# ku222/Attention-GAN

Hardware: AMD Instinct MI355X
Metric: train images/sec at 256×256 stage-3, batch 24/GPU, 1/2/4/8 MI355X (higher is better)
Workload: dtype f32; 1 GPU; full 3-stage AttnGAN 64->128->256 train step: G + 3xD updates + word attention + DAMSM words/sentence loss + KL + 4x fused Adam (BASELINE.json configs[2]); workload_key=full3, batch_per_gpu=24, global_batch=24, gf_dim=32, df_dim=64, emb_dim=256, seq_len=10, text_encoder=bypassed (frozen; N(0,1) embeddings), parallelism=dp1, discriminator_streams=3, launch=eager, gradient_exchange=none (one rank), losses_finite=True

## Files before the change

attention-gan_amd/csrc/conv.hip:

```cpp
#include "conv_common.h"

#include <cxxabi.h>
#include <cstdlib>


using namespace agan;

using namespace agan::conv;

namespace {

__global__ __launch_bounds__(256) void ktable_kernel(int2* __restrict__ tab, int n, int K, int RS, int S, int IHW, int IW, int DY) {
    const int k = blockIdx.x * 256 + threadIdx.x;
    if (k >= n) return;
    int2 a, b;
    if (k < K) {
        const int c = k / RS, rs = k - c * RS, r = rs / S, q = rs - r * S;
        const int dy = r * DY, dx = q * DY;
        a.x = c * IHW + dy * IW + dx;
        a.y = (dy & 0xFFFF) | (dx << 16);
        b.x = c * IHW * 4;
        b.y = rs * kTapRowBytes;
    } else {
        a.x = 0;
// ... 693 lines not shown
        const int kt = cdiv(K, 64);
        pack_fwd_tile(j.w, wk, j.cout, K, Nld, local % kt, local / kt, reinterpret_cast<float (*)[65]>(buf));
    } else if (j.mode == AGAN_PACK_DGRAD_S1 && j.kh * j.kw <= 16) {
        const int cg = cdiv(j.cout, kPackCo);
        pack_dgrad_tile<AGAN_PACK_DGRAD_S1>(j.w, wk, j.cout, j.cin, j.kh, j.kw, Nld, local % cg, local / cg, buf, true);
    } else if (j.mode == AGAN_PACK_DGRAD_4x4S2) {
        const int cg = cdiv(j.cout, kPackCo);
        pack_dgrad_tile<AGAN_PACK_DGRAD_4x4S2>(j.w, wk, j.cout, j.cin, j.kh, j.kw, Nld, local % cg, local / cg, buf, true);
    } else {
        const int nb = pack_job_blocks(j.mode, j.cout, j.cin, j.kh, j.kw);
        const size_t total = (size_t)ncls * K * Nld;
        for (size_t e = (size_t)local * 256 + threadIdx.x; e < total; e += (size_t)nb * 256) {
            const int n = (int)(e % Nld);
            const size_t t = e / Nld;
            wk[e] = packed_weight_value(j.w, j.mode, (int)(t / K), (int)(t % K), n, j.cout, j.cin, j.kh, j.kw);
        }
    }
}

__global__ __launch_bounds__(256) void unpack_wgrad_up_kernel(const float* __restrict__ dwk, float* __restrict__ dw, int cout, int cin,
                                                              int accumulate) {
    const int K = cin * 4;
    const size_t total = (size_t)cout * cin * 9;
    for (size_t e = (size_t)blockIdx.x * blockDim.x + threadIdx.x; e < total; e += (size_t)gridDim.x * blockDim.x) {
        const int ab = (int)(e % 9), a = ab / 3, b = ab - a * 3;
        const size_t t = e / 9;
        const int ci = (int)(t % cin), co = (int)(t / cin);
        float v = 0.f;
        for (int py = 0; py < 2; ++py)
            for (int r = 0; r < 2; ++r) {
                int rl, rh;
                up_fwd_taps(py, r, rl, rh);
                if (a < rl || a > rh) continue;
                for (int px = 0; px < 2; ++px)
                    for (int q = 0; q < 2; ++q) {
                        int sl, sh;
                        up_fwd_taps(px, q, sl, sh);
                        if (b < sl || b > sh) continue;
                        v += dwk[((size_t)(py * 2 + px) * cout + co) * K + (ci * 4 + r * 2 + q)];
                    }
            }
        dw[e] = accumulate ? dw[e] + v : v;
    }
}

__global__ __launch_bounds__(256) void bias_grad_kernel(const float* __restrict__ dy, float* __restrict__ db, int B, int C,
                                                        int HW, int accumulate) {
    __shared__ float red[4];
    const int c = blockIdx.x;
    float s = 0.f;
    for (int b = 0; b < B; ++b) {
        const float* p = dy + ((size_t)b * C + c) * HW;
        for (int i = threadIdx.x; i < HW; i += 256) s += p[i];
    }
    s = block_sum<256>(s, red);
    if (threadIdx.x == 0) db[c] = accumulate ? db[c] + s : s;
}

}

static thread_local hipEvent_t g_timer_start = nullptr, g_timer_stop = nullptr;
static thread_local const void* g_timed_kernel = nullptr;
static thread_local int g_timed_split = 0;
namespace agan { namespace conv { thread_local const void* g_noted_kernel = nullptr; } }
static inline void timer_begin(hipStream_t st) {
    if (g_timer_start) (void)hipEventRecord(g_timer_start, st);
}
static inline void timer_end(hipStream_t st, int split) {
    if (g_timer_stop) {
        (void)hipEventRecord(g_timer_stop, st);
        g_timed_kernel = agan::conv::g_noted_kernel;
        g_timed_split = split;
    }
    g_timer_start = g_timer_stop = nullptr;
}
namespace agan { namespace conv {
void timed_begin(hipStream_t st) { timer_begin(st); }
void timed_end(hipStream_t st, int split) { timer_end(st, split); }
} }

static bool dt16(int dt) { return dt == AGAN_DT_BF16 || dt == AGAN_DT_F16; }
static int mode_dtype(int mode) { return mode == AGAN_PREC_BF16 ? AGAN_DT_BF16 : (mode == AGAN_PREC_F16 ? AGAN_DT_F16 : AGAN_DT_F32); }

enum class GatherPath { none, p16, patch, winograd, small_n, direct };
struct GatherRoute {
    int mode = AGAN_PREC_F32;
    GatherPath path = GatherPath::none;
    P16Plan p16{};
    PatchPlan pp{};
    PatchGather patch{};
    WinoPlan wino{};
    GatherPlan direct{};
    size_t ws_bytes = 0;
    int split = 1;
};

static GatherRoute route_gather(const agan_conv_geom* gg, int prec, int in_dtype, int out_dtype, bool epilogue) {
    GatherRoute r;
    auto take = [&r](GatherPath path, size_t ws_bytes, int split) {
        r.path = path;
        r.ws_bytes = ws_bytes;
        r.split = split;
        return r;
    };
    if (check_geom(gg)) return r;
    const Geom g = make_geom(gg);
    if (prec_planes(prec) > 0 && patch_supported(g)) r.mode = prec;
    const bool f32io = in_dtype == AGAN_DT_F32 && out_dtype == AGAN_DT_F32;
    if (const int want = mode_dtype(r.mode)) {
        if ((in_dtype == AGAN_DT_F32 || in_dtype == want) && (out_dtype == AGAN_DT_F32 || out_dtype == want)) {
            r.p16 = plan_p16(g, in_dtype != AGAN_DT_F32);
            if (r.p16.ok) return take(GatherPath::p16, r.p16.ws_bytes, r.p16.ksplit);
        }
    }
    if (r.mode != AGAN_PREC_F32) {
        if (!f32io) return r;
        r.pp = make_patch_plan(g);
        r.patch = plan_patch_gather(g, r.pp);
        return take(GatherPath::patch, r.patch.ws_bytes, r.patch.ksplit);
    }
    if (f32io && !epilogue) {
        r.wino = plan_wino(g);
        if (r.wino.ok) return take(GatherPath::winograd, r.wino.ws_bytes, r.wino.ksplit);
    }
    if (small_n_gather_supported(g)) {
        const bool linear = g.RS == 1 && g.IH == 1 && g.IW == 1;
        if ((in_dtype == AGAN_DT_F32 || (dt16(in_dtype) && !linear)) && out_dtype == AGAN_DT_F32) return take(GatherPath::small_n, 0, 1);
        return r;
    }
    if (in_dtype == AGAN_DT_F32 && (out_dtype == AGAN_DT_F32 || dt16(out_dtype))) {
        r.direct = plan_gather(g, AGAN_PREC_F32);
        return take(GatherPath::direct, r.direct.ws_bytes, r.direct.ksplit);
    }
    return r;
}

enum class WgradPath { none, winograd, rows, patch, small_n, direct };
struct WgradRoute {
    int mode = AGAN_PREC_F32;
    WgradPath path = WgradPath::none;
    WinoWgradPlan wino{};
    RowsPlan rows{};
    PatchPlan pp{};
    PatchWgrad patch{};
    SmallWgradPlan small{};
    WgradPlan direct{};
    size_t ws_bytes = 0;
    int split = 1;
};

static WgradRoute route_wgrad(const agan_conv_geom* gg, int pack_mode, int prec, int x_dtype, int dy_dtype) {
    WgradRoute r;
    auto take = [&r](WgradPath path, size_t ws_bytes, int split) {
        r.path = path;
        r.ws_bytes = ws_bytes;
        r.split = split;
        return r;
    };
    if (check_geom(gg)) return r;
    const Geom g = make_geom(gg);
    const bool up = pack_mode == AGAN_PACK_UP_FWD, x16 = x_dtype != AGAN_DT_F32, y16 = dy_dtype != AGAN_DT_F32;
    if (prec_planes(prec) > 0 && patch_supported(g)) {
        r.mode = prec;
        if (prec == AGAN_PREC_BF16X6) r.mode = AGAN_PREC_F16X3;
        if (up && !plan_rows_wgrad(g, r.mode, false, false, true).ok) r.mode = AGAN_PREC_F32;
    }
    if (x16 || y16) {
        const int want = mode_dtype(r.mode);
        const bool ok = r.mode == AGAN_PREC_F32
                            ? pack_mode == AGAN_PACK_FWD && small_n_wgrad_supported(g) && dt16(x_dtype) && !y16
                            : want != AGAN_DT_F32 && (!x16 || x_dtype == want) && (!y16 || dy_dtype == want);
        if (!ok) return r;
    }
    if (r.mode == AGAN_PREC_F32 && !up && !x16 && !y16) {
        r.wino = plan_wino_wgrad(g);
        if (r.wino.ok) return take(WgradPath::winograd, r.wino.ws_bytes, r.wino.psplit);
    }
    if (!(r.mode == AGAN_PREC_F32 && small_n_wgrad_supported(g))) {
        r.rows = plan_rows_wgrad(g, r.mode, x16, y16, up);
        if (r.rows.ok) return take(WgradPath::rows, r.rows.ws_bytes, r.rows.psplit);
    }
    if (r.mode != AGAN_PREC_F32) {
        r.pp = make_patch_plan(g);
        r.patch = plan_patch_wgrad(g, r.pp, r.mode);
        return take(WgradPath::patch, r.patch.ws_bytes, r.patch.psplit);
    }
    if (!up && small_n_wgrad_supported(g)) {
        r.small = plan_wgrad_small_n(g);
        return take(WgradPath::small_n, r.small.ws_bytes, r.small.nchunk);
    }
    if (!x16 && !y16) {
        r.direct = plan_wgrad(g, up);
        return take(WgradPath::direct, r.direct.ws_bytes, r.direct.psplit);
    }
    return r;
}

static int check_ws(const char* who, size_t need, const void* ws, size_t ws_bytes) {
    if (need > ws_bytes || (need && !ws)) {
        set_error("%s: workspace %zu < %zu", who, ws_bytes, need);
        return AGAN_EWORKSPACE;
    }
    return AGAN_OK;
}

template <class Launch>
static int launch_main(hipStream_t st, int split, const char* what, Launch&& launch) {
    timer_begin(st);
    launch();
    timer_end(st, split);
    return check_launch(what);
}

extern "C" {

int agan_timer_last_kernel(char* name, size_t capacity) {
    AGAN_REQUIRE(name && capacity > 1, "timer_last_kernel: bad argument");
    name[0] = 0;
    if (!g_timed_kernel) return AGAN_OK;
    const char* mangled = hipKernelNameRefByPtr(g_timed_kernel, nullptr);
    if (!mangled) return AGAN_OK;
    int status = 0;
    char* dem = abi::__cxa_demangle(mangled, nullptr, nullptr, &status);
    const char* src = (status == 0 && dem) ? dem : mangled;
    strncpy(name, src, capacity - 1);
    name[capacity - 1] = 0;
    free(dem);
    return AGAN_OK;
}

int agan_timer_last_split(void) { return g_timed_kernel ? g_timed_split : 0; }

int agan_timer_create(void** event) {
    AGAN_REQUIRE(event != nullptr, "timer_create: null pointer");
    hipEvent_t e;
    if (hipEventCreate(&e) != hipSuccess) {
        set_error("timer_create: hipEventCreate failed");
        return AGAN_ELAUNCH;
    }
    *event = e;
    return AGAN_OK;
}
int agan_timer_destroy(void* event) { return (event && hipEventDestroy(static_cast<hipEvent_t>(event)) != hipSuccess) ? AGAN_ELAUNCH : AGAN_OK; }
int agan_timer_arm(void* start, void* stop) {
    g_timer_start = static_cast<hipEvent_t>(start);
    g_timer_stop = static_cast<hipEvent_t>(stop);
    return AGAN_OK;
}
int agan_timer_elapsed_ms(void* start, void* stop, float* ms) {
    AGAN_REQUIRE(start && stop && ms, "timer_elapsed_ms: null pointer");
    if (hipEventElapsedTime(ms, static_cast<hipEvent_t>(start), static_cast<hipEvent_t>(stop)) != hipSuccess) {
        set_error("timer_elapsed_ms: events not complete");
        return AGAN_ELAUNCH;
    }
    return AGAN_OK;
}

size_t agan_packed_weight_bytes(int mode, int cout, int cin, int kh, int kw, int prec) {
    int ncls, K, N;
    if (pack_dims(mode, cout, cin, kh, kw, ncls, K, N)) return 0;
    if (prec == AGAN_PREC_F32) return (size_t)ncls * K * ((N + 31) / 32 * 32) * sizeof(float);
    if (mode == AGAN_PACK_DGRAD_3x3S2) return 0;
    if (prec_planes(prec) > 0) return patch_packed_weight_bytes(mode, cout, cin, kh, kw, prec);
    return 0;
}

int agan_pack_weight(const float* w, void* wkv, int mode, int cout, int cin, int kh, int kw, int prec, void* stream) {
    int ncls, K, N;
    AGAN_REQUIRE(w && wkv, "pack_weight: null pointer");
    AGAN_REQUIRE(prec == AGAN_PREC_F32 || prec_planes(prec) > 0, "pack_weight: unknown precision mode %d", prec);
    if (prec != AGAN_PREC_F32) {
        AGAN_REQUIRE(mode != AGAN_PACK_DGRAD_3x3S2, "pack_weight: AGAN_PACK_DGRAD_3x3S2 has an fp32 layout only");
        AGAN_REQUIRE(pack_dims(mode, cout, cin, kh, kw, ncls, K, N) == 0, "pack_weight: mode %d does not take %dx%d", mode, kh, kw);
        return pack_weight_patch(w, wkv, mode, cout, cin, kh, kw, prec, as_stream(stream));
    }
    float* wk = static_cast<float*>(wkv);
    AGAN_REQUIRE(pack_dims(mode, cout, cin, kh, kw, ncls, K, N) == 0, "pack_weight: mode %d does not take %dx%d", mode, kh, kw);
    const int Nld = ((N + 31) / 32 * 32);
    const size_t total = (size_t)ncls * K * Nld;
    const int blocks = (int)std::min<size_t>(cdivz(total, 256), 8192);
    hipStream_t pst = as_stream(stream);
    if (mode == AGAN_PACK_FWD) {
        AGAN_LAUNCH(pack_fwd_tiled_kernel, dim3(cdiv(K, 64), cdiv(Nld, 64)), dim3(256), 0, pst, w, wk, cout, K, Nld);
        return check_launch("pack_weight/fwd");
    }
    if ((mode == AGAN_PACK_DGRAD_S1 && kh * kw <= 16) || mode == AGAN_PACK_DGRAD_4x4S2) {
        if (Nld != cin) (void)hipMemsetAsync(wk, 0, total * sizeof(float), pst);
        dim3 grid(cdiv(cout, kPackCo), cdiv(cin, 64));
        if (mode == AGAN_PACK_DGRAD_S1) AGAN_LAUNCH((pack_dgrad_tiled_kernel<AGAN_PACK_DGRAD_S1>), grid, dim3(256), 0, pst, w, wk, cout, cin, kh, kw, Nld);
        else AGAN_LAUNCH((pack_dgrad_tiled_kernel<AGAN_PACK_DGRAD_4x4S2>), grid, dim3(256), 0, pst, w, wk, cout, cin, kh, kw, Nld);
        return check_launch("pack_weight/dgrad");
    }
    AGAN_LAUNCH(pack_weight_kernel, dim3(blocks), dim3(256), 0, as_stream(stream), w, wk, mode, cout, cin, kh, kw, K,
                       Nld, ncls);
    return check_launch("pack_weight");
}

int agan_pack_job_blocks(int mode, int cout, int cin, int kh, int kw) { return pack_job_blocks(mode, cout, cin, kh, kw); }
int agan_pack_job_blocks_prec(int mode, int cout, int cin, int kh, int kw, int prec) {
    return prec == AGAN_PREC_F32 ? pack_job_blocks(mode, cout, cin, kh, kw) : (prec_planes(prec) > 0 ? pack_job_blocks_patch(mode, cout, cin, kh, kw) : 0);
}

int agan_pack_weights(const agan_pack_job* jobs, int njobs, int total_blocks, int prec, void* stream) {
    AGAN_REQUIRE(jobs && njobs > 0 && total_blocks > 0, "pack_weights: empty job list");
    AGAN_REQUIRE(prec == AGAN_PREC_F32 || prec_planes(prec) > 0, "pack_weights: unknown precision mode %d", prec);
    if (prec != AGAN_PREC_F32) return pack_weights_patch(jobs, njobs, total_blocks, prec, as_stream(stream));
    AGAN_LAUNCH(pack_jobs_kernel, dim3(total_blocks), dim3(256), 0, as_stream(stream), jobs, njobs);
    return check_launch("pack_weights");
}

int agan_conv_effective_prec(const agan_conv_geom* g, int prec) { return route_gather(g, prec, AGAN_DT_F32, AGAN_DT_F32, false).mode; }

int agan_conv_wgrad_effective_prec(const agan_conv_geom* g, int pack_mode, int prec) {
    return route_wgrad(g, pack_mode, prec, AGAN_DT_F32, AGAN_DT_F32).mode;
}

double agan_conv_executed_fraction(const agan_conv_geom* g, int prec, int wgrad, int plain_epilogue) {
    if (prec != AGAN_PREC_F32) return 1.0;
    if (wgrad)
        return route_wgrad(g, AGAN_PACK_FWD, prec, AGAN_DT_F32, AGAN_DT_F32).path == WgradPath::winograd ? 16.0 / 36.0 : 1.0;
    const GatherRoute r = route_gather(g, prec, AGAN_DT_F32, AGAN_DT_F32, !plain_epilogue);
    if (r.path != GatherPath::winograd) return 1.0;
    switch (r.wino.kind) {
    case WinoKind::conv4x4_s2: return 36.0 / 64.0;
    case WinoKind::dgrad2x2_class: return 9.0 / 16.0;
    case WinoKind::conv3x3:
    case WinoKind::conv3x3_half: break;
    }
    return 16.0 / 36.0;
}

static const int kDtypes[] = {AGAN_DT_F32, AGAN_DT_BF16, AGAN_DT_F16};

size_t agan_conv_gather_ws_bytes(const agan_conv_geom* g, int prec) {
    size_t a = 0;
    for (int in_dtype : kDtypes)
        for (int out_dtype : kDtypes)
            for (int epilogue = 0; epilogue < 2; ++epilogue) a = std::max(a, route_gather(g, prec, in_dtype, out_dtype, epilogue != 0).ws_bytes);
    return a;
}

size_t agan_conv_ktable_elems(const agan_conv_geom* g) {
    if (check_geom(g)) return 0;
    return (size_t)ktable_entries(g->Cin * g->R * g->S) * 4;
}

int agan_conv_ktable(const agan_conv_geom* gg, int32_t* table, void* stream) {
    if (int e = check_geom(gg)) return e;
    AGAN_REQUIRE(table != nullptr, "conv_ktable: null pointer");
    const Geom g = make_geom(gg);
    const int n = ktable_entries(g.K);
    AGAN_LAUNCH(ktable_kernel, dim3(cdiv(n, 256)), dim3(256), 0, as_stream(stream), reinterpret_cast<int2*>(table), n, g.K, g.RS,
                       g.S, g.IH * g.IW, g.IW, g.DY);
    return check_launch("conv_ktable");
}

int agan_conv_gather_dt_supported(const agan_conv_geom* gg, int prec, int in_dtype, int out_dtype) {
    return route_gather(gg, prec, in_dtype, out_dtype, false).path != GatherPath::none ? 1 : 0;
}

int agan_conv_gather_dt(const void* in_v, const void* wkv, const float* bias, void* out_v, const agan_conv_geom* gg, const int32_t* ktable,
                        int prec, int act, const void* lrelu_mask_v, void* ws, size_t ws_bytes, void* stream, const float* in_scale,
                        float* out_amax, int in_dtype, int out_dtype) {
    if (int e = check_geom(gg)) return e;
    AGAN_REQUIRE(in_v && wkv && out_v && ktable, "conv_gather: null pointer");
    AGAN_REQUIRE(act == AGAN_ACT_NONE || (act == AGAN_ACT_LRELU && gg->Cout > 4),
                 "conv_gather: fused activation %d not available for this call (MFMA paths, LeakyReLU only)", act);
    AGAN_REQUIRE(!lrelu_mask_v || (gg->Cout > 4 && act == AGAN_ACT_NONE),
                 "conv_gather: the LeakyReLU-derivative mask needs an MFMA path and no other activation");
    AGAN_REQUIRE(prec == AGAN_PREC_F32 || prec_planes(prec) > 0, "conv_gather: unknown precision mode %d", prec);
    const GatherRoute r = route_gather(gg, prec, in_dtype, out_dtype, bias || act != AGAN_ACT_NONE || lrelu_mask_v);
    AGAN_REQUIRE(r.mode == prec,
                 "conv_gather: precision mode %d does not take this geometry (agan_conv_effective_prec says which one does)", prec);
    AGAN_REQUIRE(r.path != GatherPath::none,
                 "conv_gather: 16-bit activation storage (%d -> %d) is not available for this geometry / precision %d "
                 "(agan_conv_gather_dt_supported)", in_dtype, out_dtype, prec);
    AGAN_REQUIRE(prec != AGAN_PREC_F16X3 || in_scale != nullptr, "conv_gather: AGAN_PREC_F16X3 needs the operand's agan_absmax_scale pair");
    if (int e = check_ws("conv_gather", r.ws_bytes, ws, ws_bytes)) return e;
    const Geom g = make_geom(gg);
    hipStream_t st = as_stream(stream);
    const float* in = static_cast<const float*>(in_v);
    const float* wk = static_cast<const float*>(wkv);
    const float* lrelu_mask = static_cast<const float*>(lrelu_mask_v);
    void* dst = r.split > 1 ? ws : out_v;
    const float* slabs = static_cast<const float*>(ws);
    size_t slab = 0;
    float* sum_amax = nullptr;
    int e = AGAN_OK;
    switch (r.path) {
        case GatherPath::p16:
            slab = r.p16.slab;
            e = launch_main(st, r.split, "conv_gather/p16", [&] {
                launch_p16_gather(in_v, wkv, bias, dst, g, r.p16, prec, act, lrelu_mask_v, st, in_dtype != AGAN_DT_F32, out_dtype != AGAN_DT_F32);
            });
            break;
        case GatherPath::patch:
            slab = r.patch.slab;
            sum_amax = out_amax;
            e = launch_main(st, r.split, "conv_gather/patch", [&] {
                launch_patch_gather(in, wkv, bias, static_cast<float*>(dst), g, r.pp, r.patch, prec, act, lrelu_mask, st, in_scale, out_amax);
            });
            break;
        case GatherPath::winograd:
            slab = r.wino.slab;
            slabs = reinterpret_cast<const float*>(static_cast<const char*>(ws) + r.wino.u_bytes);
            e = launch_main(st, r.split, "conv_gather/winograd", [&] { launch_wino(in, wk, static_cast<float*>(out_v), g, r.wino, ws, st); });
            break;
        case GatherPath::small_n:
            e = launch_main(st, r.split, "conv_gather/small_n", [&] { launch_gather_small_n(in_v, wk, bias, static_cast<float*>(out_v), g, st, in_dtype); });
            break;
        default: {
            const GatherPlan& p = r.direct;
            slab = p.slab;
            const int2* ktab = reinterpret_cast<const int2*>(ktable);
            e = launch_main(st, r.split, "conv_gather", [&] {
                if (p.bn == 128) launch_gather<128, 2, 2>(in, wk, bias, dst, ktab, g, p, act, lrelu_mask_v, st, out_dtype);
                else if (p.bn == 64) launch_gather<64, 2, 2>(in, wk, bias, dst, ktab, g, p, act, lrelu_mask_v, st, out_dtype);
                else launch_gather<32, 4, 1>(in, wk, bias, dst, ktab, g, p, act, lrelu_mask_v, st, out_dtype);
            });
        }
    }
    if (e || r.split == 1) return e;
    launch_sum_slabs(slabs, r.split, (size_t)g.B * g.Cout * g.OH * g.OW, slab, bias, g.Cout, g.OH * g.OW, out_v, 0, act, lrelu_mask_v, sum_amax, st,
                     out_dtype);
    return check_launch("conv_gather/sum_slabs");
}

int agan_conv_gather(const float* in, const void* wkv, const float* bias, float* out, const agan_conv_geom* gg, const int32_t* ktable,
                     int prec, int act, const float* lrelu_mask, void* ws, size_t ws_bytes, void* stream, const float* in_scale,
                     float* out_amax) {
    return agan_conv_gather_dt(in, wkv, bias, out, gg, ktable, prec, act, lrelu_mask, ws, ws_bytes, stream, in_scale, out_amax,
                               AGAN_DT_F32, AGAN_DT_F32);
}

static const int kPrecs[] = {AGAN_PREC_F32, AGAN_PREC_BF16, AGAN_PREC_BF16X3, AGAN_PREC_F16, AGAN_PREC_BF16X6, AGAN_PREC_F16X3};

size_t agan_conv_wgrad_ws_bytes(const agan_conv_geom* g) {
    if (check_geom(g)) return 0;
    const int pack_mode = g->OS == 2 ? AGAN_PACK_UP_FWD : AGAN_PACK_FWD;
    size_t a = 0;
    for (int prec : kPrecs)
        for (int x_dtype : kDtypes)
            for (int dy_dtype : kDtypes) a = std::max(a, route_wgrad(g, pack_mode, prec, x_dtype, dy_dtype).ws_bytes);
    return a;
}

int agan_conv_wgrad_dt_supported(const agan_conv_geom* gg, int pack_mode, int prec, int x_dtype, int dy_dtype) {
    return route_wgrad(gg, pack_mode, prec, x_dtype, dy_dtype).path != WgradPath::none ? 1 : 0;
}

int agan_conv_wgrad(const float* x, const float* dy, float* dw, const agan_conv_geom* gg, const int32_t* ktable, int pack_mode,
                    int kh, int kw, int prec, int accumulate, void* ws, size_t ws_bytes, void* stream, const float* x_scale,
                    const float* dy_scale) {
    return agan_conv_wgrad_dt(x, dy, dw, gg, ktable, pack_mode, kh, kw, prec, accumulate, ws, ws_bytes, stream, x_scale, dy_scale,
                              AGAN_DT_F32, AGAN_DT_F32);
}

int agan_conv_wgrad_dt(const void* x_v, const void* dy_v, float* dw, const agan_conv_geom* gg, const int32_t* ktable, int pack_mode,
                       int kh, int kw, int prec, int accumulate, void* ws, size_t ws_bytes, void* stream, const float* x_scale,
                       const float* dy_scale, int x_dtype, int dy_dtype) {
    const WgradRoute r = route_wgrad(gg, pack_mode, prec, x_dtype, dy_dtype);
    AGAN_REQUIRE(r.path != WgradPath::none,
                 "conv_wgrad: 16-bit activation storage (%d, %d) is not available for this geometry / precision %d", x_dtype, dy_dtype, prec);
    AGAN_REQUIRE(x_v && dy_v && dw && ktable, "conv_wgrad: null pointer");
    AGAN_REQUIRE(prec == AGAN_PREC_F32 || prec_planes(prec) > 0, "conv_wgrad: unknown precision mode %d", prec);
    AGAN_REQUIRE(pack_mode == AGAN_PACK_FWD || pack_mode == AGAN_PACK_UP_FWD, "conv_wgrad: pack mode %d is not a forward mode", pack_mode);
    const Geom g = make_geom(gg);
    const bool up = pack_mode == AGAN_PACK_UP_FWD;
    AGAN_REQUIRE(1LL * g.B * g.Cin * g.IH * g.IW < (1LL << 29) && 1LL * g.B * g.Cout * g.OH * g.OW < (1LL << 29),
                 "conv_wgrad: tensor exceeds 2^29 elements");
    if (!up) AGAN_REQUIRE(g.R == kh && g.S == kw && g.OS == 1, "conv_wgrad: geometry is not a direct %dx%d conv", kh, kw);
    else AGAN_REQUIRE(g.R == 2 && g.S == 2 && g.OS == 2 && kh == 3 && kw == 3, "conv_wgrad: geometry is not the folded upsample conv");
    AGAN_REQUIRE(r.mode != AGAN_PREC_F16X3 || (x_scale && dy_scale),
                 "conv_wgrad: precision mode %d runs this weight gradient as AGAN_PREC_F16X3 (agan_conv_wgrad_effective_prec), which needs the "
                 "amax slots of x and dy (x_amax / dy_amax)", prec);
    if (int e = check_ws("conv_wgrad", r.ws_bytes, ws, ws_bytes)) return e;
    hipStream_t st = as_stream(stream);
    const float* x = static_cast<const float*>(x_v);
    const float* dy = static_cast<const float*>(dy_v);
    float* wsf = static_cast<float*>(ws);
    const bool x16 = x_dtype != AGAN_DT_F32, y16 = dy_dtype != AGAN_DT_F32;
    switch (r.path) {
        case WgradPath::winograd:
            if (int e = launch_main(st, r.split, "conv_wgrad/winograd", [&] { launch_wino_wgrad(x, dy, wsf, g, r.wino, st); })) return e;
            launch_wino_wgrad_sum(wsf, g, r.wino, dw, accumulate ? 1 : 0, st);
            return check_launch("conv_wgrad/winograd/sum");
        case WgradPath::rows:
        case WgradPath::patch: {
            const bool rows = r.path == WgradPath::rows;
            int e;
            if (rows) e = launch_main(st, r.split, "conv_wgrad/rows", [&] {
                launch_rows_wgrad(x_v, dy_v, wsf, g, r.rows, r.mode, st, x_scale, dy_scale, x16, y16);
            });
            else e = launch_main(st, r.split, "conv_wgrad/patch", [&] {
                launch_patch_wgrad(x_v, dy_v, wsf, g, r.pp, r.patch, r.mode, st, x_scale, dy_scale, x16, y16);
            });
            if (e) return e;
            const size_t slab = rows ? r.rows.slab : r.patch.slab;
            const int NPH = rows ? r.rows.NPH : r.pp.NPH, NT = rows ? r.rows.NT : r.pp.NT, Kp = rows ? r.rows.Kp : r.patch.Kp;
            const int ncls = rows ? 1 : r.patch.ncls;
            const bool unfold = up && !rows;
            float* reduced = r.split > 1 ? wsf + slab * r.split : wsf;
            const bool sum_first = unfold ? r.split > 1 : r.split > 4;
            if (sum_first) {
                launch_sum_slabs(wsf, r.split, (size_t)ncls * g.Cout * Kp, slab, nullptr, 1, 1, reduced, 0, AGAN_ACT_NONE, nullptr, nullptr, st);
                if (int e2 = check_launch("conv_wgrad/sum_slabs")) return e2;
            }
            if (unfold) launch_patch_wgrad_unpack(reduced, dw, g.Cout, g.Cin, kh, kw, up, r.pp, r.patch, accumulate, st);
            else launch_wgrad_sum_unpack(sum_first ? reduced : wsf, sum_first ? 1 : r.split, slab, dw, g.Cout, g.Cin, kh, kw, NPH, NT, Kp, accumulate, st);
            return check_launch("conv_wgrad/unpack");
        }
        case WgradPath::small_n: {
            if (int e = launch_main(st, r.split, "conv_wgrad/small_n", [&] { launch_wgrad_small_n(x_v, dy, wsf, g, r.small, st, x_dtype); })) return e;
            launch_sum_slabs(wsf, r.split, (size_t)g.Cout * g.K, r.small.slab, nullptr, 1, 1, dw, accumulate, AGAN_ACT_NONE, nullptr, nullptr, st);
            return check_launch("conv_wgrad/small_n/sum_slabs");
        }
        default: {
            const WgradPlan& p = r.direct;
            const int acc_in_kernel = (accumulate && !up && p.psplit == 1) ? 1 : 0;
            const bool via_sum = p.psplit > 1 || (accumulate && !up && !acc_in_kernel);
            float* reduced = up ? wsf + (p.psplit > 1 ? p.slab * p.psplit : 0) : dw;
            float* part = via_sum ? wsf : reduced;
            const int2* ktab = reinterpret_cast<const int2*>(ktable);
            dim3 grid(p.itiles, p.jtiles, p.ncls * p.psplit);
#define AGAN_WG(BI, BJ) AGAN_LAUNCH((conv_wgrad_f32_kernel<BI, BJ>), grid, dim3(256), 0, st, x, dy, part, ktab, g, p.psplit, p.pchunk, p.slab, acc_in_kernel)
            const int e = launch_main(st, r.split, "conv_wgrad", [&] {
                if (p.bi == 128 && p.bj == 128) AGAN_WG(128, 128);
                else if (p.bi == 128) AGAN_WG(128, 64);
                else if (p.bj == 128) AGAN_WG(64, 128);
                else AGAN_WG(64, 64);
            });
#undef AGAN_WG
            if (e) return e;
            if (via_sum) {
                launch_sum_slabs(part, p.psplit, (size_t)p.ncls * g.Cout * g.K, p.slab, nullptr, 1, 1, reduced, (accumulate && !up) ? 1 : 0,
                                 AGAN_ACT_NONE, nullptr, nullptr, st);
                if (int e2 = check_launch("conv_wgrad/sum_slabs")) return e2;
            }
            if (up) {
                const size_t total = (size_t)g.Cout * g.Cin * 9;
                AGAN_LAUNCH(unpack_wgrad_up_kernel, dim3((unsigned)std::min<size_t>(cdivz(total, 256), 4096)), dim3(256), 0, st,
                            reduced, dw, g.Cout, g.Cin, accumulate);
                return check_launch("conv_wgrad/unpack");
            }
            return AGAN_OK;
        }
    }
}

int agan_bias_grad(const float* dy, float* dbias, int B, int C, int HW, int accumulate, void* stream) {
    AGAN_REQUIRE(dy && dbias && B > 0 && C > 0 && HW > 0, "bias_grad: bad argument");
    AGAN_LAUNCH(bias_grad_kernel, dim3(C), dim3(256), 0, as_stream(stream), dy, dbias, B, C, HW, accumulate);
    return check_launch("bias_grad");
}

static int conv2d_geom(const agan_conv2d_desc* d, int dgrad, Geom& g, int& pack_mode) {
    AGAN_REQUIRE(d != nullptr, "conv2d: null descriptor");
    AGAN_REQUIRE(d->B > 0 && d->Cin > 0 && d->IH > 0 && d->IW > 0 && d->Cout > 0 && d->OH > 0 && d->OW > 0, "conv2d: non-positive dimension");
    AGAN_REQUIRE(d->KH > 0 && d->KW > 0 && d->KH * d->KW <= kMaxTaps2d, "conv2d: %dx%d taps unsupported (at most %d)", d->KH, d->KW, kMaxTaps2d);
    AGAN_REQUIRE((d->SH == 1 || d->SH == 2) && (d->SW == 1 || d->SW == 2), "conv2d: strides %dx%d unsupported (1 or 2 per axis)", d->SH, d->SW);
    AGAN_REQUIRE(d->PH >= 0 && d->PW >= 0 && d->PH < d->KH && d->PW < d->KW, "conv2d: padding %dx%d unsupported for %dx%d taps", d->PH, d->PW,
                 d->KH, d->KW);
    AGAN_REQUIRE(d->OH == (d->IH + 2 * d->PH - d->KH) / d->SH + 1 && d->OW == (d->IW + 2 * d->PW - d->KW) / d->SW + 1 &&
                     d->IH + 2 * d->PH >= d->KH && d->IW + 2 * d->PW >= d->KW,
                 "conv2d: output %dx%d does not match input %dx%d, taps %dx%d, stride %dx%d, padding %dx%d", d->OH, d->OW, d->IH, d->IW, d->KH,
                 d->KW, d->SH, d->SW, d->PH, d->PW);
    AGAN_REQUIRE(d->in_c0 >= 0 && d->in_c0 + d->Cin <= d->in_ctot && d->out_c0 >= 0 && d->out_c0 + d->Cout <= d->out_ctot,
                 "conv2d: channel slice out of range (in %d+%d of %d, out %d+%d of %d)", d->in_c0, d->Cin, d->in_ctot, d->out_c0, d->Cout,
                 d->out_ctot);
    const long long xe = 1LL * d->B * d->in_ctot * d->IH * d->IW, ye = 1LL * d->B * d->out_ctot * d->OH * d->OW;
    AGAN_REQUIRE(xe < (1LL << 30) && ye < (1LL << 30), "conv2d: tensor exceeds 2^30 elements (32-bit buffer offsets)");
    Geom& r = g;
    r = Geom{};
    r.B = d->B;
    r.DY = 1;
    const int xhw = d->IH * d->IW, yhw = d->OH * d->OW;
    if (!dgrad) {
        r.Cin = d->Cin; r.IH = d->IH; r.IW = d->IW; r.Cout = d->Cout; r.OH = d->OH; r.OW = d->OW;
        r.R = d->KH; r.S = d->KW; r.OS = 1; r.SY = d->SH; r.SX = d->SW;
        r.OY0 = r.OY1 = -d->PH; r.OX0 = r.OX1 = -d->PW;
        r.in0 = d->in_c0 * xhw; r.inB = d->in_ctot * xhw; r.out0 = d->out_c0 * yhw; r.outB = d->out_ctot * yhw;
        pack_mode = AGAN_PACK_FWD;
    } else {
        r.Cin = d->Cout; r.IH = d->OH; r.IW = d->OW; r.Cout = d->Cin; r.OH = d->IH; r.OW = d->IW;
        r.in0 = d->out_c0 * yhw; r.inB = d->out_ctot * yhw; r.out0 = d->in_c0 * xhw; r.outB = d->in_ctot * xhw;
        r.SY = r.SX = 1;
        if (d->SH == 1 && d->SW == 1) {
            r.R = d->KH; r.S = d->KW; r.OS = 1;
            r.OY0 = r.OY1 = -(d->KH - 1 - d->PH); r.OX0 = r.OX1 = -(d->KW - 1 - d->PW);
            pack_mode = AGAN_PACK_DGRAD_S1;
        } else {
            AGAN_REQUIRE(d->SH == 2 && d->SW == 2 && d->KH == 3 && d->KW == 3 && d->PH == 0 && d->PW == 0,
                         "conv2d: no data-gradient decomposition for %dx%d taps, stride %dx%d, padding %dx%d (stride 2: 3x3 unpadded only)",
                         d->KH, d->KW, d->SH, d->SW, d->PH, d->PW);
// ... 78 lines not shown
```

attention-gan_amd/csrc/conv_common.h:

```cpp
#pragma once
#include "agan_common.h"

#include <algorithm>
#include <type_traits>

namespace agan {
namespace conv {

typedef float f32x16 __attribute__((ext_vector_type(16)));

extern thread_local const void* g_noted_kernel;
#define AGAN_LAUNCH(kernel, ...)                                                   \
    do {                                                                           \
        ::agan::conv::g_noted_kernel = reinterpret_cast<const void*>(kernel);      \
        hipLaunchKernelGGL(kernel, __VA_ARGS__);                                   \
    } while (0)
void timed_begin(hipStream_t st);
void timed_end(hipStream_t st, int split);


struct FastDiv {
    unsigned mul, shift;
    __device__ __forceinline__ int div(int n) const { return (int)((__umulhi(mul, (unsigned)n) + (unsigned)n) >> shift); }
};
// ... 128 lines not shown
__host__ __device__ inline int pack_dims(int mode, int cout, int cin, int kh, int kw, int& ncls, int& K, int& N) {
    switch (mode) {
        case AGAN_PACK_FWD: ncls = 1; K = cin * kh * kw; N = cout; return 0;
        case AGAN_PACK_DGRAD_S1: ncls = 1; K = cout * kh * kw; N = cin; return 0;
        case AGAN_PACK_DGRAD_4x4S2: if (kh != 4 || kw != 4) return -1; ncls = 4; K = cout * 4; N = cin; return 0;
        case AGAN_PACK_UP_FWD: if (kh != 3 || kw != 3) return -1; ncls = 4; K = cin * 4; N = cout; return 0;
        case AGAN_PACK_UP_DGRAD: if (kh != 3 || kw != 3) return -1; ncls = 1; K = cout * 16; N = cin; return 0;
        case AGAN_PACK_DGRAD_3x3S2: if (kh != 3 || kw != 3) return -1; ncls = 4; K = cout * 4; N = cin; return 0;
    }
    return -1;
}

__device__ __forceinline__ int linear_block_id() { return blockIdx.x + gridDim.x * (blockIdx.y + gridDim.y * blockIdx.z); }
__device__ __forceinline__ int xcd_contiguous(int L, int T) {
    const int xcd = L & 7, idx = L >> 3;
    int start = 0;
    for (int i = 0; i < xcd; ++i) start += (T - i + 7) >> 3;
    return start + idx;
}

struct GatherPlan {
    int bn, mtiles, ntiles, ncls, ksplit, kchunk;
    size_t slab, ws_bytes;
};

inline GatherPlan plan_gather(const Geom& g, int prec) {
    const int bk = prec == AGAN_PREC_F32 ? 16 : 32;
    const int slots = prec == AGAN_PREC_F32 ? 768 : 512;
    GatherPlan p;
    p.bn = g.Cout >= 96 ? 128 : (g.Cout >= 48 ? 64 : 32);
    p.mtiles = cdiv(g.Mtot, 128);
    p.ntiles = cdiv(g.Cout, p.bn);
    p.ncls = g.OS * g.OS;
    const int tiles = p.mtiles * p.ntiles * p.ncls;
    const int ktiles = cdiv(g.K, bk);
    int ks = 1;
    if (tiles < slots) ks = std::max(1, std::min({slots / tiles, std::max(1, ktiles / 16), 32}));
    p.kchunk = cdiv(ktiles, ks) * bk;
    p.ksplit = cdiv(g.K, p.kchunk);
    p.slab = (size_t)g.B * g.Cout * g.OH * g.OW;
    p.slab = (p.slab + 3) / 4 * 4;
    p.ws_bytes = p.ksplit > 1 ? p.slab * p.ksplit * sizeof(float) : 0;
    return p;
}

struct WgradPlan {
    int bi, bj, itiles, jtiles, ncls, psplit, pchunk;
    size_t slab, ws_bytes;
};

inline WgradPlan plan_wgrad(const Geom& g, bool needs_combine) {
    WgradPlan p;
    p.bi = (g.K >= 96 && cdiv(g.K, 128) * 128 <= cdiv(g.K, 64) * 64) ? 128 : 64;
    p.bj = g.Cout >= 96 ? 128 : 64;
    p.itiles = cdiv(g.K, p.bi);
    p.jtiles = cdiv(g.Cout, p.bj);
    p.ncls = g.OS * g.OS;
    const int tiles = p.itiles * p.jtiles * p.ncls;
    const int ptiles = cdiv(g.Mtot, 32);
    int ps = 1;
    if (tiles < 512) {
        const int cap = std::max(1, ptiles / 4);
        const int ps1 = std::max(1, std::min(512 / tiles, cap)), ps2 = std::max(1, std::min(1024 / tiles, cap));
        const double fill1 = (double)tiles * ps1 / 512.0, fill2 = (double)tiles * ps2 / 1024.0;
        ps = std::min(fill2 > fill1 + 1e-9 ? ps2 : ps1, 2048);
    }
    p.pchunk = cdiv(ptiles, ps) * 32;
    p.psplit = cdiv(g.Mtot, p.pchunk);
    p.slab = ((size_t)p.ncls * g.Cout * g.K + 3) / 4 * 4;
    const size_t nslabs = p.psplit + (needs_combine ? 1 : 0);
    p.ws_bytes = p.slab * nslabs * sizeof(float);
    return p;
}

struct SmallWgradPlan {
    int pchunk, nchunk;
    size_t slab, ws_bytes;
};
bool small_n_gather_supported(const Geom& g);
void launch_gather_small_n(const void* in, const float* wk, const float* bias, float* out, const Geom& g, hipStream_t st, int in_dtype = AGAN_DT_F32);
bool small_n_wgrad_supported(const Geom& g);
SmallWgradPlan plan_wgrad_small_n(const Geom& g);
void launch_wgrad_small_n(const void* x, const float* dy, float* part, const Geom& g, const SmallWgradPlan& p, hipStream_t st, int x_dtype = AGAN_DT_F32);

__host__ __device__ inline void pack_taps(int mode, int kh, int kw, int& R, int& S, int& SY) {
    switch (mode) {
        case AGAN_PACK_DGRAD_4x4S2: case AGAN_PACK_UP_FWD: R = S = 2; SY = 1; return;
        case AGAN_PACK_UP_DGRAD: R = S = 4; SY = 2; return;
        default: R = kh; S = kw; SY = (kh == 4) ? 2 : 1; return;
    }
}
struct PatchPlan {
    int twl, thl;
    int tiles_x, tiles_y, tiles_b, mtiles;
    int PW, PH, PHW, PP;
    int NPH, NT, IS;
    int nchunks, nstages, nsteps;
    int tapoff[9];
    int tappos[9];
    int base_y[2][2], base_x[2][2];
    FastDiv dPP, dPHW, dPW;
    FastDiv dNT, dNCLS, dMT, dTX, dTY, dNPH, dNPH2;
    int g_ntiles, g_ncls;
};
struct PatchGather {
    int bn, ntiles, ncls, ksplit, stages_per_split;
    size_t slab, ws_bytes;
};
struct PatchWgrad {
    int bj, jtiles, ncls, psplit, tiles_per_split, Kp;
    size_t slab, ws_bytes;
};
struct P16Plan {
    int ok;
    int gk;
    int twl, thl, TB;
    int tiles_x, tiles_y, tiles_b, mtiles;
    int PH, PW, LW, NXB, PXB, CHS;
    int nitems, NI;
    int nstages, wsteps;
    int bn, ntiles, ncls, ksplit, stages_per_split;
    int buf_bytes, smem_bytes;
    int lds_epi;
    int px2;
    int wc, lp;
    size_t slab, ws_bytes;
    FastDiv dNXB, dPH, dTB, dNT, dNCLS, dMT, dTX, dTY;
};
P16Plan plan_p16(const Geom& g, bool in16);
void launch_p16_gather(const void* in, const void* wk, const float* bias, void* dst, const Geom& g, const P16Plan& p, int prec, int act,
                       const void* lrelu_mask, hipStream_t st, bool in16, bool out16);
struct RowsPlan {
    int ok, gk, ci2, ups;
    int twl, thl, tbl;
    int tiles_x, tiles_y, tiles_b, mtiles;
    int XR, XRT;
    int rowb, cpitch;
    int halo, NBY, drowb, dpitch;
    int plane_bytes, smem_bytes, pc;
    int nxbl, nxitems, nyitems;
    int bj, jtiles, nchunks, ngroups, psplit, tiles_per_split;
    int NPH, NT, Kp;
    size_t slab, ws_bytes;
    FastDiv dXRT, dXR, dNBY;
};
enum class WinoKind : int {
    conv3x3,
    conv3x3_half,
    conv4x4_s2,
    dgrad2x2_class,
};
struct WinoPlan {
    int ok;
    WinoKind kind;
    int txl, tyl;
    int blocks_x, blocks_y, blocks_b, mtiles;
    int nf, ntiles;
    int pcp, raw_items, raw_bytes;
    int mpc, mpr;
    int smem_bytes;
    int ksplit, chunks_per_split;
    size_t u_bytes, slab, ws_bytes;
};
struct WinoWgradPlan {
    int ok, noct, jtiles, itiles, psplit, octs_per_split, smem_bytes;
    size_t slab, ws_bytes;
// ... 34 lines not shown
```

Before: 1001 images/s.

## Add skinny fully-connected forward and weight-gradient kernels for small batch

Adds a dedicated path for 1x1-spatial convolutions (linear layers such as the noise/condition FC and the attention projections) with small batch M. The forward kernel stages the whole input batch in LDS, streams weight columns per lane, and splits K across waves and blocks, with an optional combine kernel. The wgrad kernel holds x in registers and writes dW directly with no split-slab workspace. It is meant to replace the generic small_n and direct tiles, which underuse the GPU on tall-skinny GEMMs. In exchange it adds routing complexity and a distinct epilogue class (bias allowed, activation not).

```diff
diff --git a/attention-gan_amd/csrc/conv.hip b/attention-gan_amd/csrc/conv.hip
--- a/attention-gan_amd/csrc/conv.hip
+++ b/attention-gan_amd/csrc/conv.hip
@@ -799,7 +799,7 @@
 static bool dt16(int dt) { return dt == AGAN_DT_BF16 || dt == AGAN_DT_F16; }
 static int mode_dtype(int mode) { return mode == AGAN_PREC_BF16 ? AGAN_DT_BF16 : (mode == AGAN_PREC_F16 ? AGAN_DT_F16 : AGAN_DT_F32); }
 
-enum class GatherPath { none, p16, patch, winograd, small_n, direct };
+enum class GatherPath { none, p16, patch, winograd, skinny, small_n, direct };
 struct GatherRoute {
     int mode = AGAN_PREC_F32;
     GatherPath path = GatherPath::none;
@@ -807,12 +807,14 @@
     PatchPlan pp{};
     PatchGather patch{};
     WinoPlan wino{};
+    SkinnyGatherPlan skinny{};
     GatherPlan direct{};
     size_t ws_bytes = 0;
     int split = 1;
 };
 
-static GatherRoute route_gather(const agan_conv_geom* gg, int prec, int in_dtype, int out_dtype, bool epilogue) {
+enum { kEpiNone = 0, kEpiBias = 1, kEpiAct = 2 };
+static GatherRoute route_gather(const agan_conv_geom* gg, int prec, int in_dtype, int out_dtype, int epilogue) {
     GatherRoute r;
     auto take = [&r](GatherPath path, size_t ws_bytes, int split) {
         r.path = path;
@@ -836,9 +838,13 @@
         r.patch = plan_patch_gather(g, r.pp);
         return take(GatherPath::patch, r.patch.ws_bytes, r.patch.ksplit);
     }
-    if (f32io && !epilogue) {
+    if (f32io && epilogue == kEpiNone) {
         r.wino = plan_wino(g);
         if (r.wino.ok) return take(GatherPath::winograd, r.wino.ws_bytes, r.wino.ksplit);
+    }
+    if (f32io && epilogue != kEpiAct && skinny_gather_supported(g)) {
+        r.skinny = plan_gather_skinny(g);
+        return take(GatherPath::skinny, r.skinny.ws_bytes, r.skinny.ksplit);
     }
     if (small_n_gather_supported(g)) {
         const bool linear = g.RS == 1 && g.IH == 1 && g.IW == 1;
@@ -852,7 +858,7 @@
     return r;
 }
 
-enum class WgradPath { none, winograd, rows, patch, small_n, direct };
+enum class WgradPath { none, winograd, rows, patch, skinny, small_n, direct };
 struct WgradRoute {
     int mode = AGAN_PREC_F32;
     WgradPath path = WgradPath::none;
@@ -860,6 +866,7 @@
     RowsPlan rows{};
     PatchPlan pp{};
     PatchWgrad patch{};
+    SkinnyWgradPlan skinny{};
     SmallWgradPlan small{};
     WgradPlan direct{};
     size_t ws_bytes = 0;
@@ -902,6 +909,10 @@
         r.patch = plan_patch_wgrad(g, r.pp, r.mode);
         return take(WgradPath::patch, r.patch.ws_bytes, r.patch.psplit);
     }
+    if (!up && !x16 && !y16 && skinny_wgrad_supported(g)) {
+        r.skinny = plan_wgrad_skinny(g);
+        return take(WgradPath::skinny, 0, 1);
+    }
     if (!up && small_n_wgrad_supported(g)) {
         r.small = plan_wgrad_small_n(g);
         return take(WgradPath::small_n, r.small.ws_bytes, r.small.nchunk);
@@ -1026,7 +1037,7 @@
     return check_launch("pack_weights");
 }
 
-int agan_conv_effective_prec(const agan_conv_geom* g, int prec) { return route_gather(g, prec, AGAN_DT_F32, AGAN_DT_F32, false).mode; }
+int agan_conv_effective_prec(const agan_conv_geom* g, int prec) { return route_gather(g, prec, AGAN_DT_F32, AGAN_DT_F32, kEpiNone).mode; }
 
 int agan_conv_wgrad_effective_prec(const agan_conv_geom* g, int pack_mode, int prec) {
     return route_wgrad(g, pack_mode, prec, AGAN_DT_F32, AGAN_DT_F32).mode;
@@ -1036,7 +1047,7 @@
     if (prec != AGAN_PREC_F32) return 1.0;
     if (wgrad)
         return route_wgrad(g, AGAN_PACK_FWD, prec, AGAN_DT_F32, AGAN_DT_F32).path == WgradPath::winograd ? 16.0 / 36.0 : 1.0;
-    const GatherRoute r = route_gather(g, prec, AGAN_DT_F32, AGAN_DT_F32, !plain_epilogue);
+    const GatherRoute r = route_gather(g, prec, AGAN_DT_F32, AGAN_DT_F32, plain_epilogue ? kEpiNone : kEpiAct);
     if (r.path != GatherPath::winograd) return 1.0;
     switch (r.wino.kind) {
     case WinoKind::conv4x4_s2: return 36.0 / 64.0;
@@ -1053,7 +1064,7 @@
     size_t a = 0;
     for (int in_dtype : kDtypes)
         for (int out_dtype : kDtypes)
-            for (int epilogue = 0; epilogue < 2; ++epilogue) a = std::max(a, route_gather(g, prec, in_dtype, out_dtype, epilogue != 0).ws_bytes);
+            for (int epilogue = kEpiNone; epilogue <= kEpiAct; ++epilogue) a = std::max(a, route_gather(g, prec, in_dtype, out_dtype, epilogue).ws_bytes);
     return a;
 }
 
@@ -1073,7 +1084,7 @@
 }
 
 int agan_conv_gather_dt_supported(const agan_conv_geom* gg, int prec, int in_dtype, int out_dtype) {
-    return route_gather(gg, prec, in_dtype, out_dtype, false).path != GatherPath::none ? 1 : 0;
+    return route_gather(gg, prec, in_dtype, out_dtype, kEpiNone).path != GatherPath::none ? 1 : 0;
 }
 
 int agan_conv_gather_dt(const void* in_v, const void* wkv, const float* bias, void* out_v, const agan_conv_geom* gg, const int32_t* ktable,
@@ -1086,7 +1097,8 @@
     AGAN_REQUIRE(!lrelu_mask_v || (gg->Cout > 4 && act == AGAN_ACT_NONE),
                  "conv_gather: the LeakyReLU-derivative mask needs an MFMA path and no other activation");
     AGAN_REQUIRE(prec == AGAN_PREC_F32 || prec_planes(prec) > 0, "conv_gather: unknown precision mode %d", prec);
-    const GatherRoute r = route_gather(gg, prec, in_dtype, out_dtype, bias || act != AGAN_ACT_NONE || lrelu_mask_v);
+    const GatherRoute r = route_gather(gg, prec, in_dtype, out_dtype,
+                                       (act != AGAN_ACT_NONE || lrelu_mask_v) ? kEpiAct : (bias ? kEpiBias : kEpiNone));
     AGAN_REQUIRE(r.mode == prec,
                  "conv_gather: precision mode %d does not take this geometry (agan_conv_effective_prec says which one does)", prec);
     AGAN_REQUIRE(r.path != GatherPath::none,
@@ -1123,6 +1135,13 @@
             slabs = reinterpret_cast<const float*>(static_cast<const char*>(ws) + r.wino.u_bytes);
             e = launch_main(st, r.split, "conv_gather/winograd", [&] { launch_wino(in, wk, static_cast<float*>(out_v), g, r.wino, ws, st); });
             break;
+        case GatherPath::skinny:
+            e = launch_main(st, r.split, "conv_gather/skinny", [&] {
+                launch_gather_skinny(in, wk, bias, static_cast<float*>(out_v), static_cast<float*>(ws), g, r.skinny, st);
+            });
+            if (e || r.split == 1) return e;
+            launch_gather_skinny_combine(slabs, bias, static_cast<float*>(out_v), g, r.skinny, st);
+            return check_launch("conv_gather/skinny/combine");
         case GatherPath::small_n:
             e = launch_main(st, r.split, "conv_gather/small_n", [&] { launch_gather_small_n(in_v, wk, bias, static_cast<float*>(out_v), g, st, in_dtype); });
             break;
@@ -1227,6 +1246,8 @@
             else launch_wgrad_sum_unpack(sum_first ? reduced : wsf, sum_first ? 1 : r.split, slab, dw, g.Cout, g.Cin, kh, kw, NPH, NT, Kp, accumulate, st);
             return check_launch("conv_wgrad/unpack");
         }
+        case WgradPath::skinny:
+            return launch_main(st, r.split, "conv_wgrad/skinny", [&] { launch_wgrad_skinny(x, dy, dw, g, r.skinny, accumulate ? 1 : 0, st); });
         case WgradPath::small_n: {
             if (int e = launch_main(st, r.split, "conv_wgrad/small_n", [&] { launch_wgrad_small_n(x_v, dy, wsf, g, r.small, st, x_dtype); })) return e;
             launch_sum_slabs(wsf, r.split, (size_t)g.Cout * g.K, r.small.slab, nullptr, 1, 1, dw, accumulate, AGAN_ACT_NONE, nullptr, nullptr, st);
diff --git a/attention-gan_amd/csrc/conv_common.h b/attention-gan_amd/csrc/conv_common.h
--- a/attention-gan_amd/csrc/conv_common.h
+++ b/attention-gan_amd/csrc/conv_common.h
@@ -234,6 +234,21 @@
 bool small_n_wgrad_supported(const Geom& g);
 SmallWgradPlan plan_wgrad_small_n(const Geom& g);
 void launch_wgrad_small_n(const void* x, const float* dy, float* part, const Geom& g, const SmallWgradPlan& p, hipStream_t st, int x_dtype = AGAN_DT_F32);
+struct SkinnyGatherPlan {
+    int mt, mblocks, cgroups, nwk, ksplit, kchunk;
+    size_t slab, ws_bytes, lds_bytes;
+};
+struct SkinnyWgradPlan {
+    int mt, ktiles, nchunk, nchunks;
+};
+bool skinny_gather_supported(const Geom& g);
+SkinnyGatherPlan plan_gather_skinny(const Geom& g);
+void launch_gather_skinny(const float* in, const float* wk, const float* bias, float* out, float* part, const Geom& g, const SkinnyGatherPlan& p,
+                          hipStream_t st);
+void launch_gather_skinny_combine(const float* part, const float* bias, float* out, const Geom& g, const SkinnyGatherPlan& p, hipStream_t st);
+bool skinny_wgrad_supported(const Geom& g);
+SkinnyWgradPlan plan_wgrad_skinny(const Geom& g);
+void launch_wgrad_skinny(const float* x, const float* dy, float* dw, const Geom& g, const SkinnyWgradPlan& p, int accumulate, hipStream_t st);
 
 __host__ __device__ inline void pack_taps(int mode, int kh, int kw, int& R, int& S, int& SY) {
     switch (mode) {
diff --git a/attention-gan_amd/csrc/conv_skinny.hip b/attention-gan_amd/csrc/conv_skinny.hip
--- /dev/null
+++ b/attention-gan_amd/csrc/conv_skinny.hip
@@ -0,0 +1,224 @@
+#include "conv_common.h"
+
+using namespace agan;
+using namespace agan::conv;
+
+namespace {
+
+constexpr int kRowBatch = 16;
+constexpr int kGatherLds = 64 * 1024;
+constexpr int kHeadMinK = 64;
+
+template <int MT>
+__global__ __launch_bounds__(512) void skinny_small_n_gather_kernel(const float* __restrict__ in, const float* __restrict__ wk,
+                                                                    const float* __restrict__ bias, float* __restrict__ dst, int M, int K,
+                                                                    int N, int Nld, int kchunk) {
+    extern __shared__ __attribute__((aligned(16))) float smem[];
+    constexpr int LD = MT + 4;
+    const int lane = threadIdx.x & 63, w = threadIdx.x >> 6, nwk = blockDim.x >> 6;
+    const int n = blockIdx.x * 64 + lane;
+    const int k0 = blockIdx.y * kchunk, kn = min(kchunk, K - k0);
+    const int m0 = blockIdx.z * MT, mn = min(MT, M - m0);
+    const int rpw = cdiv(kn, nwk), kb = w * rpw, ke = min(kn, kb + rpw);
+    const bool nok = n < Nld;
+    const float* wp = wk + (size_t)k0 * Nld + (nok ? n : 0);
+    float wv[kRowBatch];
+#pragma unroll
+    for (int j = 0; j < kRowBatch; ++j) wv[j] = (nok && kb + j < ke) ? wp[(size_t)(kb + j) * Nld] : 0.f;
+    for (int i = threadIdx.x; i < kn * (MT / 4); i += blockDim.x) {
+        const int m4 = i / kn, k = i - m4 * kn;
+        float v[4];
+#pragma unroll
+        for (int j = 0; j < 4; ++j) {
+            const int m = m4 * 4 + j;
+            v[j] = m < mn ? in[(size_t)(m0 + m) * K + k0 + k] : 0.f;
+        }
+        *reinterpret_cast<float4*>(smem + k * LD + m4 * 4) = make_float4(v[0], v[1], v[2], v[3]);
+    }
+    __syncthreads();
+    float acc[MT];
+#pragma unroll
+    for (int m = 0; m < MT; ++m) acc[m] = 0.f;
+    for (int r = kb; r < ke; r += kRowBatch) {
+        float wn[kRowBatch];
+#pragma unroll
+        for (int j = 0; j < kRowBatch; ++j) wn[j] = (nok && r + kRowBatch + j < ke) ? wp[(size_t)(r + kRowBatch + j) * Nld] : 0.f;
+#pragma unroll
+        for (int j = 0; j < kRowBatch; ++j) {
+            if (r + j < ke) {
+                const float4* xr = reinterpret_cast<const float4*>(smem + (r + j) * LD);
+#pragma unroll
+                for (int q = 0; q < MT / 4; ++q) {
+                    const float4 xv = xr[q];
+                    acc[4 * q + 0] += xv.x * wv[j];
+                    acc[4 * q + 1] += xv.y * wv[j];
+                    acc[4 * q + 2] += xv.z * wv[j];
+                    acc[4 * q + 3] += xv.w * wv[j];
+                }
+            }
+        }
+#pragma unroll
+        for (int j = 0; j < kRowBatch; ++j) wv[j] = wn[j];
+    }
+    if (nwk > 1) {
+        __syncthreads();
+        if (w > 0) {
+#pragma unroll
+            for (int m = 0; m < MT; ++m) smem[((w - 1) * MT + m) * 64 + lane] = acc[m];
+        }
+        __syncthreads();
+        if (w == 0) {
+            for (int v = 1; v < nwk; ++v) {
+#pragma unroll
+                for (int m = 0; m < MT; ++m) acc[m] += smem[((v - 1) * MT + m) * 64 + lane];
+            }
+        }
+    }
+    if (w == 0 && n < N) {
+        const float bv = bias ? bias[n] : 0.f;
+        float* o = dst + ((size_t)blockIdx.y * M + m0) * N + n;
+#pragma unroll
+        for (int m = 0; m < MT; ++m)
+            if (m < mn) o[(size_t)m * N] = acc[m] + bv;
+    }
+}
+
+__global__ __launch_bounds__(256) void skinny_small_n_combine_kernel(const float* __restrict__ part, const float* __restrict__ bias,
+                                                                     float* __restrict__ out, int total, int N, int nsplit) {
+    const int e = blockIdx.x * 256 + threadIdx.x;
+    if (e >= total) return;
+    float s = 0.f;
+    for (int i0 = 0; i0 < nsplit; i0 += 16) {
+        float v[16];
+#pragma unroll
+        for (int j = 0; j < 16; ++j) v[j] = i0 + j < nsplit ? part[(size_t)(i0 + j) * total + e] : 0.f;
+#pragma unroll
+        for (int h = 1; h < 16; h *= 2)
+#pragma unroll
+            for (int j = 0; j < 16; j += 2 * h) v[j] += v[j + h];
+        s += v[0];
+    }
+    out[e] = s + (bias ? bias[e % N] : 0.f);
+}
+
+template <int MT>
+__global__ __launch_bounds__(256) void skinny_small_n_wgrad_kernel(const float* __restrict__ x, const float* __restrict__ dy,
+                                                                   float* __restrict__ dw, int M, int K, int N, int nchunk, int accumulate) {
+    const int lane = threadIdx.x & 63, w = __builtin_amdgcn_readfirstlane(threadIdx.x >> 6);
+    __shared__ __attribute__((aligned(16))) float sdy[MT * 64];
+    const int k = (blockIdx.x * 4 + w) * 64 + lane;
+    const bool kok = k < K;
+    const int n0 = blockIdx.y * nchunk, nn = min(nchunk, N - n0);
+    float xr[MT];
+#pragma unroll
+    for (int m = 0; m < MT; ++m) xr[m] = (kok && m < M) ? x[(size_t)m * K + k] : 0.f;
+    for (int i = threadIdx.x; i < MT * nchunk; i += 256) {
+        const int m = i / nchunk, j = i - m * nchunk;
+        sdy[i] = (m < M && j < nn) ? dy[(size_t)m * N + n0 + j] : 0.f;
+    }
+    __syncthreads();
+    if (k - lane >= K) return;
+    for (int nb = 0; nb < nn; nb += 8) {
+        float acc[8];
+#pragma unroll
+        for (int j = 0; j < 8; ++j) acc[j] = 0.f;
+#pragma unroll
+        for (int m = 0; m < MT; ++m) {
+            const float4* d = reinterpret_cast<const float4*>(sdy + m * nchunk + nb);
+            const float4 a = d[0], b = d[1];
+            acc[0] += xr[m] * a.x; acc[1] += xr[m] * a.y; acc[2] += xr[m] * a.z; acc[3] += xr[m] * a.w;
+            acc[4] += xr[m] * b.x; acc[5] += xr[m] * b.y; acc[6] += xr[m] * b.z; acc[7] += xr[m] * b.w;
+            if ((m & 3) == 3)
+                asm volatile("" : "+v"(acc[0]), "+v"(acc[1]), "+v"(acc[2]), "+v"(acc[3]), "+v"(acc[4]), "+v"(acc[5]), "+v"(acc[6]), "+v"(acc[7])
+                             :: "memory");
+        }
+        if (kok) {
+#pragma unroll
+            for (int j = 0; j < 8; ++j) {
+                if (nb + j < nn) {
+                    const size_t e = (size_t)(n0 + nb + j) * K + k;
+                    dw[e] = accumulate ? dw[e] + acc[j] : acc[j];
+                }
+            }
+        }
+    }
+}
+
+bool skinny_geometry(const Geom& g) {
+    return g.IH == 1 && g.IW == 1 && g.OH == 1 && g.OW == 1 && g.R == 1 && g.S == 1 && g.OS == 1 && g.SY == 1 && g.OY0 == 0;
+}
+
+}
+
+namespace agan {
+namespace conv {
+
+bool skinny_gather_supported(const Geom& g) {
+    return skinny_geometry(g) && !(g.Cout <= 4 && g.K < kHeadMinK);
+}
+
+SkinnyGatherPlan plan_gather_skinny(const Geom& g) {
+    SkinnyGatherPlan p;
+    const int M = g.B;
+    p.mblocks = cdiv(M, 32);
+    p.mt = std::max(8, agan_round_up(cdiv(M, p.mblocks), 8));
+    p.cgroups = cdiv(g.Nld, 64);
+    const int kmax = kGatherLds / ((p.mt + 4) * 4) / 8 * 8;
+    int ks = 1;
+    if (g.K > kmax) ks = std::max(cdiv(g.K, kmax), std::min({256 / std::min(256, p.cgroups * p.mblocks), cdiv(g.K, 32), 64}));
+    p.kchunk = agan_round_up(cdiv(g.K, ks), 8);
+    p.ksplit = cdiv(g.K, p.kchunk);
+    p.nwk = std::max(1, std::min(8, cdiv(std::min(p.kchunk, g.K), 4)));
+    p.lds_bytes = sizeof(float) * std::max((size_t)p.kchunk * (p.mt + 4), (size_t)(p.nwk - 1) * p.mt * 64);
+    p.slab = (size_t)M * g.Cout;
+    p.ws_bytes = p.ksplit > 1 ? p.slab * p.ksplit * sizeof(float) : 0;
+    return p;
+}
+
+void launch_gather_skinny(const float* in, const float* wk, const float* bias, float* out, float* part, const Geom& g, const SkinnyGatherPlan& p,
+                          hipStream_t st) {
+    const bool split = p.ksplit > 1;
+    const dim3 grid(p.cgroups, p.ksplit, p.mblocks), block(64 * p.nwk);
+#define AGAN_SK(MT_)                                                                                                       \
+    AGAN_LAUNCH((skinny_small_n_gather_kernel<MT_>), grid, block, p.lds_bytes, st, in, wk, split ? nullptr : bias, split ? part : out, g.B, \
+                g.K, g.Cout, g.Nld, p.kchunk)
+    switch (p.mt) {
+        case 8: AGAN_SK(8); break;
+        case 16: AGAN_SK(16); break;
+        case 24: AGAN_SK(24); break;
+        default: AGAN_SK(32); break;
+    }
+#undef AGAN_SK
+}
+
+void launch_gather_skinny_combine(const float* part, const float* bias, float* out, const Geom& g, const SkinnyGatherPlan& p, hipStream_t st) {
+    const int total = (int)p.slab;
+    AGAN_LAUNCH(skinny_small_n_combine_kernel, dim3(cdiv(total, 256)), dim3(256), 0, st, part, bias, out, total, g.Cout, p.ksplit);
+}
+
+bool skinny_wgrad_supported(const Geom& g) { return skinny_geometry(g) && g.B <= 64; }
+
+SkinnyWgradPlan plan_wgrad_skinny(const Geom& g) {
+    SkinnyWgradPlan p;
+    p.mt = g.B <= 8 ? 8 : (g.B <= 24 ? 24 : (g.B <= 48 ? 48 : 64));
+    p.ktiles = cdiv(g.K, 256);
+    p.nchunk = std::max(8, std::min(64, agan_round_up(cdiv(g.Cout * p.ktiles, 512), 8)));
+    p.nchunks = cdiv(g.Cout, p.nchunk);
+    return p;
+}
+
+void launch_wgrad_skinny(const float* x, const float* dy, float* dw, const Geom& g, const SkinnyWgradPlan& p, int accumulate, hipStream_t st) {
+    const dim3 grid(p.ktiles, p.nchunks);
+#define AGAN_SK(MT_) \
+    AGAN_LAUNCH((skinny_small_n_wgrad_kernel<MT_>), grid, dim3(256), 0, st, x, dy, dw, g.B, g.K, g.Cout, p.nchunk, accumulate)
+    switch (p.mt) {
+        case 8: AGAN_SK(8); break;
+        case 24: AGAN_SK(24); break;
+        case 48: AGAN_SK(48); break;
+        default: AGAN_SK(64); break;
+    }
+#undef AGAN_SK
+}
+
+}
+}
```

Measured after the change: 1006 images/s (median of 6 runs). Within noise of the previous version (+0.4%).
